# 5l1v3r1/PBS

Measured on AMD Instinct MI355X. Metric: co-run slowdown (%) vs solo + aggregate throughput, 4-tenant mix at 1/2/4/8 GPU, higher is better.
Workload: dtype bf16

## Files before the change

csrc/hip/tenant_kernels.hip:

```cpp
#include "common.hpp"

namespace gpbs_hip {


__device__ __forceinline__ int grab_unit_x(WorkQueue* q, const PartTable* table, u32 mode, u32 me, u32 xcc,
                                           int* s_slot, u32 total) {
  if (threadIdx.x == 0) {
    int u = -1;
    hold_wait(table, mode);
    const u32 per = (total + kXcds - 1) / kXcds;
    for (u32 spins = 0;; ++spins) {
      if (owns(table, mode, me, xcc)) {
        for (u32 k = 0; k < (u32)kXcds; ++k) {
          const u32 r = (xcc + k) & (kXcds - 1);
          const u32 lo = r * per, hi = min(lo + per, total);
          if (lo >= hi) continue;
          if (__hip_atomic_load(&q->xnext[r], __ATOMIC_RELAXED, __HIP_MEMORY_SCOPE_AGENT) >= hi - lo) continue;
          const u32 t = atomicAdd(&q->xnext[r], 1u);
          if (t < hi - lo) {
            u = (int)(lo + t);
            atomicAdd(&q->next, 1u);
            break;
          }
        }
        break;
      }
      if ((mode & 3) != GATE_PARK || spins >= kParkSpins ||
          __hip_atomic_load(&q->next, __ATOMIC_RELAXED, __HIP_MEMORY_SCOPE_AGENT) >= total) {
        atomicAdd(&q->stopped, 1u);
        break;
      }
#pragma unroll
      for (int k = 0; k < 6; ++k) __builtin_amdgcn_s_sleep(127);
    }
    *s_slot = u;
  }
  __syncthreads();
  int u = *s_slot;
  __syncthreads();
  return u;
}


__device__ __forceinline__ u16 f2bf(float x) { return __builtin_bit_cast(u16, (__bf16)x); }
__device__ __forceinline__ float bf2f(u16 x) { return __uint_as_float(((u32)x) << 16); }

constexpr int GBM = 128, GBN = 128, GBK = 64, GNT = 256;
constexpr int kGemmLds = 2 * 2 * GBM * GBK * 2;

typedef __attribute__((address_space(3))) char lds_t;

__device__ __forceinline__ void glds16(const void* g, lds_t* l) {
  __builtin_amdgcn_global_load_lds(g, (__attribute__((address_space(3))) void*)l, 16, 0, 0);
}

__global__ __launch_bounds__(GNT, 2) void k_gemm_bf16_tn(const u16* __restrict__ A, const u16* __restrict__ Bt,
                                                         u16* __restrict__ C, int M, int N, int K, WorkQueue* q,
                                                         const PartTable* table, u32 mode, u32 me, u64* cnt,
                                                         u32 inst_per_tile, u32 refs_per_tile, u32 miss_per_tile,
                                                         u32* status) {
  __shared__ __attribute__((aligned(16))) char smem[kGemmLds + 16];
  lds_t* lds = (lds_t*)smem;
  int* s_slot = (int*)(smem + kGemmLds);
  const u32 xcc = xcc_id();
  u64 t_last = __builtin_amdgcn_s_memtime();
  const int tid = threadIdx.x, lane = tid & 63, wid = tid >> 6;
  const int wr = wid >> 1, wc = wid & 1;
  const int tiles_m = M / GBM, tiles_n = N / GBN, ntiles = tiles_m * tiles_n;
  const int nk = K / GBK;
  constexpr int GROUP_M = 8;

  int srow[4], scol[4];
#pragma unroll
  for (int j = 0; j < 4; ++j) {
    const int c = wid * 4 + j;
    srow[j] = 8 * c + (lane >> 3);
    scol[j] = (((lane & 7) ^ (srow[j] & 7)) * 8);
  }

  for (;;) {
    const int t = grab_unit(q, table, mode, me, xcc, s_slot, (u32)ntiles);
    if (t < 0) break;
    const int in_group = GROUP_M * tiles_n;
    const int g = t / in_group;
    const int first_m = g * GROUP_M;
    const int gsz = min(tiles_m - first_m, GROUP_M);
    const int tm = first_m + (t % in_group) % gsz;
    const int tn = (t % in_group) / gsz;
    const u16* Ab = A + (size_t)tm * GBM * K;
    const u16* Bb = Bt + (size_t)tn * GBN * K;

    f32x4 acc[4][4];
#pragma unroll
    for (int i = 0; i < 4; ++i)
#pragma unroll
      for (int j = 0; j < 4; ++j) acc[i][j] = f32x4{0.f, 0.f, 0.f, 0.f};

    auto stage = [&](int buf, int kt) {
      lds_t* la = lds + buf * (2 * GBM * GBK * 2);
      lds_t* lb = la + GBM * GBK * 2;
#pragma unroll
      for (int j = 0; j < 4; ++j) {
        const int c = wid * 4 + j;
        glds16(Ab + (size_t)srow[j] * K + kt * GBK + scol[j], la + c * 1024);
        glds16(Bb + (size_t)srow[j] * K + kt * GBK + scol[j], lb + c * 1024);
      }
    };

    stage(0, 0);
    asm volatile("s_waitcnt vmcnt(0)" ::: "memory");
    __syncthreads();
    int cur = 0;
    for (int kt = 0; kt < nk; ++kt) {
      if (kt + 1 < nk) stage(cur ^ 1, kt + 1);
      const lds_t* la = lds + cur * (2 * GBM * GBK * 2);
      const lds_t* lb = la + GBM * GBK * 2;
#pragma unroll
      for (int s = 0; s < 2; ++s) {
        bf16x8 a[4], b[4];
        const int chunk = s * 4 + (lane >> 4);
#pragma unroll
        for (int i = 0; i < 4; ++i) {
          const int ra = wr * 64 + i * 16 + (lane & 15);
          a[i] = *(const __attribute__((address_space(3))) bf16x8*)(la + ra * 128 + ((chunk ^ (ra & 7)) << 4));
          const int rb = wc * 64 + i * 16 + (lane & 15);
          b[i] = *(const __attribute__((address_space(3))) bf16x8*)(lb + rb * 128 + ((chunk ^ (rb & 7)) << 4));
        }
#pragma unroll
        for (int i = 0; i < 4; ++i)
#pragma unroll
          for (int j = 0; j < 4; ++j) acc[i][j] = __builtin_amdgcn_mfma_f32_16x16x32_bf16(a[i], b[j], acc[i][j], 0, 0, 0);
      }
      asm volatile("s_waitcnt vmcnt(0)" ::: "memory");
      __syncthreads();
      cur ^= 1;
    }
#pragma unroll
    for (int i = 0; i < 4; ++i)
#pragma unroll
      for (int j = 0; j < 4; ++j) {
        const int m = tm * GBM + wr * 64 + i * 16 + (lane >> 4) * 4;
        const int n = tn * GBN + wc * 64 + j * 16 + (lane & 15);
#pragma unroll
        for (int r = 0; r < 4; ++r) C[(size_t)(m + r) * N + n] = f2bf(acc[i][j][r]);
      }
    count_unit(cnt, me, xcc, inst_per_tile, &t_last, refs_per_tile, miss_per_tile, q);
  }
  finish(q, status, (u32)ntiles);
}

constexpr int G2_BM = 256, G2_BK = 64, G2_NT = 512;
constexpr u32 kGemmXRange = 1u << 16;
constexpr u32 kGemmBlock2D = 1u << 17;
constexpr u32 kGemmStatic = 1u << 18;
constexpr int kGemmOptsLive = 1 | 8 | 1 << 23;
constexpr int kGemmOptsShipped = 256 | 8192 | 65536 | 131072;
static int g_gemm_opts = 8;
constexpr int kG2Half = 128 * 128;
constexpr int kG2Buf = 4 * kG2Half;
constexpr int kG2Lds = 2 * kG2Buf;

__device__ __forceinline__ int g2_swz(int r) { return (r >> 1) & 7; }

__global__ __launch_bounds__(G2_NT, 1) void k_gemm256_bf16_tn(const u16* __restrict__ A, const u16* __restrict__ Bt,
                                                             u16* __restrict__ C, int M, int N, int K, WorkQueue* q,
                                                             const PartTable* table, u32 mode, u32 me, u64* cnt,
                                                             u32 inst_per_tile, u32 refs_per_tile, u32 miss_per_tile,
                                                             u32* status) {
  __shared__ __attribute__((aligned(16))) char smem[kG2Lds + 16];
  lds_t* lds = (lds_t*)smem;
  int* s_slot = (int*)(smem + kG2Lds);
  const u32 xcc = xcc_id();
  u64 t_last = __builtin_amdgcn_s_memtime();
  const int tid = threadIdx.x, lane = tid & 63, wid = tid >> 6;
  const int wu = __builtin_amdgcn_readfirstlane(wid);
  const int wr = wu >> 2, wc = wu & 3;
  const int tiles_m = M / G2_BM, tiles_n = N / G2_BM, ntiles = tiles_m * tiles_n;
  const int nt = K / G2_BK;
  int soff[2];
#pragma unroll
  for (int j = 0; j < 2; ++j) {
    const int row = 8 * (2 * wid + j) + (lane >> 3);
    soff[j] = row * K + (((lane & 7) ^ g2_swz(row)) * 8);
  }
  int soffa[4];
#pragma unroll
  for (int j = 0; j < 4; ++j) {
    const int row = 8 * (4 * (wid & 3) + j) + (lane >> 3);
    soffa[j] = row * K + (((lane & 7) ^ g2_swz(row)) * 8);
  }
  const int l16 = lane & 15, lq = lane >> 4;
  const int bh = wc >> 1, bc = (wc & 1) * 64;
  int units_seen = 0;

  for (;;) {
    const int tile = (mode & kGemmStatic) ? (units_seen ? -1 : (int)blockIdx.x)
                     : (mode & kGemmXRange) ? grab_unit_x(q, table, mode, me, xcc, s_slot, (u32)ntiles)
                                            : grab_unit(q, table, mode, me, xcc, s_slot, (u32)ntiles);
    if (tile < 0) break;
    int tm = tile / tiles_n, tn = tile % tiles_n;
    if ((mode & kGemmBlock2D) && (tiles_m & 3) == 0 && (tiles_n & 1) == 0 && ntiles % kXcds == 0) {
      const int per = ntiles / kXcds;
      const int bm = tiles_m / 4, bn = tiles_n / 2;
      const int g = (mode & kGemmXRange) ? tile / per : tile % kXcds;
      const int jj = (mode & kGemmXRange) ? tile % per : tile / kXcds;
      tm = (g >> 1) * bm + jj / bn;
      tn = (g & 1) * bn + jj % bn;
    }
    const u16* Ab = A + (size_t)tm * G2_BM * K;
    const u16* Bb = Bt + (size_t)tn * G2_BM * K;
    auto stage = [&](int kind, int h, int t) {
      const u16* src = (kind ? Bb : Ab) + (size_t)h * 128 * K + t * G2_BK;
      lds_t* dst = lds + (t & 1) * kG2Buf + (kind * 2 + h) * kG2Half + wid * 2048;
      glds16(src + soff[0], dst);
      glds16(src + soff[1], dst + 1024);
    };
    auto stage_own_a = [&](int t) {
      const u16* src = Ab + (size_t)wr * 128 * K + t * G2_BK;
      lds_t* dst = lds + (t & 1) * kG2Buf + wr * kG2Half + (wid & 3) * 4096;
#pragma unroll
      for (int j = 0; j < 4; ++j) glds16(src + soffa[j], dst + j * 1024);
    };
    auto frag = [&](int b, int kind, int h, int r0, int s) -> bf16x8 {
      const int r = r0 + l16;
      const lds_t* p = lds + b * kG2Buf + (kind * 2 + h) * kG2Half + r * 128 + (((4 * s + lq) ^ g2_swz(r)) << 4);
      return *(const __attribute__((address_space(3))) bf16x8*)p;
    };
    f32x4 acc[8][4];
#pragma unroll
    for (int i = 0; i < 8; ++i)
#pragma unroll
      for (int j = 0; j < 4; ++j) acc[i][j] = f32x4{0.f, 0.f, 0.f, 0.f};
    stage(1, 0, 0); stage(1, 1, 0); stage(0, 0, 0); stage(0, 1, 0);
    asm volatile("s_waitcnt vmcnt(0)" ::: "memory");
    __builtin_amdgcn_s_barrier();
    if (wr == 1) __builtin_amdgcn_s_barrier();
    bf16x8 a[4][2], b[4][2];
    for (int t = 0; t < nt; ++t) {
      const int buf = t & 1;
      const bool more = t + 1 < nt;
#pragma unroll
      for (int j = 0; j < 4; ++j)
#pragma unroll
        for (int s2 = 0; s2 < 2; ++s2) b[j][s2] = frag(buf, 1, bh, bc + j * 16, s2);
      __builtin_amdgcn_sched_barrier(0);
#pragma unroll
      for (int i = 0; i < 4; ++i)
#pragma unroll
        for (int s2 = 0; s2 < 2; ++s2) a[i][s2] = frag(buf, 0, wr, i * 16, s2);
      if (more) {
        stage(1, 0, t + 1); stage(1, 1, t + 1);
      } else {
        asm volatile("s_waitcnt vmcnt(0)" ::: "memory");
      }
      __builtin_amdgcn_s_barrier();
      asm volatile("s_waitcnt lgkmcnt(0)" ::: "memory");
      __builtin_amdgcn_s_setprio(1);
#pragma unroll
      for (int s2 = 0; s2 < 2; ++s2)
#pragma unroll
        for (int i = 0; i < 4; ++i)
#pragma unroll
          for (int j = 0; j < 4; ++j)
            acc[i][j] = __builtin_amdgcn_mfma_f32_16x16x32_bf16(b[j][s2], a[i][s2], acc[i][j], 0, 0, 0);
      __builtin_amdgcn_s_setprio(0);
      __builtin_amdgcn_s_barrier();
#pragma unroll
      for (int i = 0; i < 4; ++i)
#pragma unroll
        for (int s2 = 0; s2 < 2; ++s2) a[i][s2] = frag(buf, 0, wr, 64 + i * 16, s2);
      if (more) {
        stage_own_a(t + 1);
        asm volatile("s_waitcnt vmcnt(4)" ::: "memory");
      }
      __builtin_amdgcn_s_barrier();
      asm volatile("s_waitcnt lgkmcnt(0)" ::: "memory");
      __builtin_amdgcn_s_setprio(1);
#pragma unroll
      for (int s2 = 0; s2 < 2; ++s2)
#pragma unroll
        for (int i = 0; i < 4; ++i)
#pragma unroll
          for (int j = 0; j < 4; ++j)
            acc[4 + i][j] = __builtin_amdgcn_mfma_f32_16x16x32_bf16(b[j][s2], a[i][s2], acc[4 + i][j], 0, 0, 0);
      __builtin_amdgcn_s_setprio(0);
      asm volatile("s_waitcnt vmcnt(0)" ::: "memory");
      __builtin_amdgcn_s_barrier();
    }
    if (wr == 0) __builtin_amdgcn_s_barrier();
#pragma unroll
    for (int i = 0; i < 8; ++i)
#pragma unroll
      for (int j = 0; j < 4; ++j) {
        const int m = wr * 128 + i * 16 + l16;
        const int c8 = wc * 16 + j * 4 + lq;
        const u32 lo = (u32)f2bf(acc[i][j][0]) | ((u32)f2bf(acc[i][j][1]) << 16);
        const u32 hi = (u32)f2bf(acc[i][j][2]) | ((u32)f2bf(acc[i][j][3]) << 16);
        *(__attribute__((address_space(3))) u32x2*)(lds + m * 512 + ((c8 ^ (m & 15)) << 3)) = u32x2{lo, hi};
      }
    __syncthreads();
#pragma unroll
    for (int p = 0; p < 16; ++p) {
      const int row = p * 16 + (tid >> 5), c16 = tid & 31;
      u32x4 v = *(const __attribute__((address_space(3))) u32x4*)(lds + row * 512 + (((2 * c16) ^ (row & 14)) << 3));
      if (row & 1) v = u32x4{v.z, v.w, v.x, v.y};
      u32x4* dst = (u32x4*)(C + (size_t)(tm * G2_BM + row) * N + tn * G2_BM + c16 * 8);
      __builtin_nontemporal_store(v, dst);
    }
    __syncthreads();
    ++units_seen;
    if (!(mode & kGemmStatic)) count_unit(cnt, me, xcc, inst_per_tile, &t_last, refs_per_tile, miss_per_tile, q);
  }
  if (!(mode & kGemmStatic)) finish(q, status, (u32)ntiles);
}

constexpr int SNT = 256, SUNROLL = 16, RUNROLL = 6;

template <int U, bool NTS>
__global__ __launch_bounds__(SNT) void k_stream_copy(const f32x4* __restrict__ src, f32x4* __restrict__ dst,
                                                    u64 n4, u32 chunk4, WorkQueue* q, const PartTable* table, u32 mode,
                                                    u32 me, u64* cnt, u32* status) {
  __shared__ int s_slot[4];
  const u32 xcc = xcc_id();
  u64 t_last = __builtin_amdgcn_s_memtime();
  const u32 nchunks = (u32)((n4 + chunk4 - 1) / chunk4);
  const u64 lines = (u64)chunk4 * 16 / 128;
  const u64 inst = (u64)chunk4 * 2 / 64 + 8;
  for (;;) {
    const int c = grab_unit(q, table, mode, me, xcc, s_slot, nchunks);
    if (c < 0) break;
    const u64 base = (u64)c * chunk4;
    const u64 end = min(base + chunk4, n4);
    for (u64 i = base + threadIdx.x; i < end; i += (u64)SNT * U) {
      f32x4 v[U];
#pragma unroll
      for (int k = 0; k < U; ++k) {
        const u64 idx = i + (u64)k * SNT;
        if (idx < end) v[k] = __builtin_nontemporal_load(src + idx);
      }
#pragma unroll
      for (int k = 0; k < U; ++k) {
        const u64 idx = i + (u64)k * SNT;
        if (idx < end) {
          if constexpr (NTS)
            __builtin_nontemporal_store(v[k], dst + idx);
          else
            dst[idx] = v[k];
        }
      }
    }
    count_unit(cnt, me, xcc, inst, &t_last, 2 * lines, 2 * lines, q);
  }
  finish(q, status, nchunks);
}

template <int NT, int U, bool NTL, bool NTS>
__global__ __launch_bounds__(NT) void k_reduce_bf16(const u32x4* __restrict__ a, const u32x4* __restrict__ b,
                                                    u32x4* __restrict__ out, u64 n8, u32 chunk8, WorkQueue* q,
                                                    const PartTable* table, u32 mode, u32 me, u64* cnt,
                                                    u32* status) {
  __shared__ int s_slot[4];
  const u32 xcc = xcc_id();
  u64 t_last = __builtin_amdgcn_s_memtime();
  const u32 nchunks = (u32)((n8 + chunk8 - 1) / chunk8);
  const u64 lines = (u64)chunk8 * 16 / 128;
  const u64 inst = (u64)chunk8 * 3 / 64 + (u64)chunk8 * 16 / 64;
  for (;;) {
    const int c = grab_unit(q, table, mode, me, xcc, s_slot, nchunks);
    if (c < 0) break;
    const u64 base = (u64)c * chunk8, end = min(base + chunk8, n8);
    for (u64 i = base + threadIdx.x; i < end; i += (u64)NT * U) {
      u32x4 x[U], y[U];
#pragma unroll
      for (int k = 0; k < U; ++k) {
        const u64 idx = i + (u64)k * NT;
        if (idx < end) {
          if constexpr (NTL) {
            x[k] = __builtin_nontemporal_load(a + idx);
            y[k] = __builtin_nontemporal_load(b + idx);
          } else {
            x[k] = a[idx];
            y[k] = b[idx];
          }
        }
      }
#pragma unroll
      for (int k = 0; k < U; ++k) {
        const u64 idx = i + (u64)k * NT;
        if (idx >= end) continue;
        const u32* px = (const u32*)&x[k];
        const u32* py = (const u32*)&y[k];
        u32x4 r;
        u32* pr = (u32*)&r;
#pragma unroll
        for (int w = 0; w < 4; ++w) {
          const float lo = bf2f((u16)(px[w] & 0xffff)) + bf2f((u16)(py[w] & 0xffff));
          const float hi = bf2f((u16)(px[w] >> 16)) + bf2f((u16)(py[w] >> 16));
          pr[w] = (u32)f2bf(lo) | ((u32)f2bf(hi) << 16);
        }
        if constexpr (NTS)
          __builtin_nontemporal_store(r, out + idx);
        else
          out[idx] = r;
      }
    }
    count_unit(cnt, me, xcc, inst, &t_last, 3 * lines, 3 * lines, q);
  }
  finish(q, status, nchunks);
}

constexpr int GV_U = 2;

__device__ __forceinline__ float dot8(const u32x4 w, const u32x4 v) {
  float s = 0.f;
#pragma unroll
  for (int e = 0; e < 4; ++e) {
    s += __uint_as_float(w[e] << 16) * __uint_as_float(v[e] << 16);
    s += __uint_as_float(w[e] & 0xffff0000u) * __uint_as_float(v[e] & 0xffff0000u);
  }
  return s;
}

__global__ __launch_bounds__(256) __attribute__((amdgpu_waves_per_eu(5, 8))) void k_gemv_bf16(const u16* __restrict__ W, const u16* __restrict__ x,
                                                  float* __restrict__ y, int R, int K, WorkQueue* q,
                                                  const PartTable* table, u32 mode, u32 me, u64* cnt,
                                                  u32* status) {
  __shared__ int s_slot[4];
  if (mode & GATE_WAVEPRIO) __builtin_amdgcn_s_setprio(3);
  const u32 xcc = xcc_id();
  u64 t_last = __builtin_amdgcn_s_memtime();
  const int lane = threadIdx.x & 63, wid = threadIdx.x >> 6;
  const u32 nchunks = (u32)((R + 15) / 16);
  const u64 lines = (u64)16 * K * 2 / 128;
  const int nk = K / 512;
  const u32x4* xv = (const u32x4*)x;
  for (;;) {
    const int c = grab_unit(q, table, mode, me, xcc, s_slot, nchunks);
    if (c < 0) break;
    const int row0 = c * 16 + wid * 4;
    const u32x4* wr[4];
#pragma unroll
    for (int r = 0; r < 4; ++r) wr[r] = (const u32x4*)(W + (size_t)min(row0 + r, R - 1) * K);
    float acc[4] = {0.f, 0.f, 0.f, 0.f};
    int kc = 0;
    for (; kc + GV_U <= nk; kc += GV_U) {
      u32x4 xr[GV_U], wv[GV_U][4];
#pragma unroll
      for (int u = 0; u < GV_U; ++u) {
        const int k = (kc + u) * 64 + lane;
        xr[u] = xv[k];
#pragma unroll
        for (int r = 0; r < 4; ++r) wv[u][r] = __builtin_nontemporal_load(wr[r] + k);
      }
#pragma unroll
      for (int u = 0; u < GV_U; ++u)
#pragma unroll
        for (int r = 0; r < 4; ++r) acc[r] += dot8(wv[u][r], xr[u]);
    }
    for (; kc < nk; ++kc) {
      const int k = kc * 64 + lane;
      const u32x4 xr = xv[k];
#pragma unroll
      for (int r = 0; r < 4; ++r) acc[r] += dot8(__builtin_nontemporal_load(wr[r] + k), xr);
    }
#pragma unroll
    for (int r = 0; r < 4; ++r) {
      float s = acc[r];
#pragma unroll
      for (int off = 32; off > 0; off >>= 1) s += __shfl_xor(s, off, 64);
      if (lane == 0 && row0 + r < R) y[row0 + r] = s;
    }
    count_unit(cnt, me, xcc, (u64)16 * (K / 512 + 8), &t_last, lines, lines, q);
  }
  finish(q, status, nchunks);
}

__global__ void k_census(u32* out, const PartTable* table, u32 mode, u32 me) {
  const u32 xcc = xcc_id();
  const bool ok = owns(table, mode, me, xcc);
  if (threadIdx.x == 0) {
    out[blockIdx.x * 4 + 0] = xcc;
    out[blockIdx.x * 4 + 1] = hw_id();
    out[blockIdx.x * 4 + 2] = ok ? 1u : 0u;
    out[blockIdx.x * 4 + 3] = 0xC0FFEEu;
  }
  if (ok) {
    u64 t = __builtin_amdgcn_s_memtime();
    while (__builtin_amdgcn_s_memtime() - t < 2000) __builtin_amdgcn_s_sleep(1);
  }
}

}

using namespace gpbs_hip;

extern "C" {

int gpbs_hip_set_gemm_opts(int opts) {
  const int old = g_gemm_opts;
  if (opts < 0) return old;
  const int gone = opts & ~(kGemmOptsLive | kGemmOptsShipped);
  static bool warned = false;
  if (gone && !warned) {
    warned = true;
    fprintf(stderr,
            "gpbs_hip_set_gemm_opts: bits 0x%x select GEMM variants that were removed (docs/gemm_lab.md); "
            "the shipped schedule runs\n",
            gone);
  }
  g_gemm_opts = opts & kGemmOptsLive;
  return old;
}

int gpbs_hip_gemm_units(int M, int N) {
  if (M % G2_BM == 0 && N % G2_BM == 0) return (M / G2_BM) * (N / G2_BM);
  return (M / GBM) * (N / GBN);
}

int gpbs_hip_gemm_bf16(const void* A, const void* Bt, void* C, int M, int N, int K, void* q, const void* table,
                       unsigned mode, unsigned me, void* cnt, void* status, int grid, hipStream_t s) {
  if (M % GBM || N % GBN || K % GBK || M <= 0 || N <= 0 || K <= 0) return -22;
  if (M % G2_BM == 0 && N % G2_BM == 0) {
    const int ntiles = (M / G2_BM) * (N / G2_BM);
    if (grid <= 0) grid = 256;
    if (grid > ntiles) grid = ntiles;
    const u32 inst = (u32)((G2_BM / 16) * (G2_BM / 16) * (K / 32) + (K / G2_BK) * 64 + 128);
    const u32 refs = (u32)(((u64)2 * G2_BM * K * 2) / 128);
    const u32 miss = (u32)((((u64)M + N) * K * 2 / 128) / ntiles + (u64)G2_BM * G2_BM * 2 / 128);
    const u32 m2 = mode | ((g_gemm_opts & 1) ? kGemmXRange : 0u) |
                   ((g_gemm_opts & 8) && ntiles % kXcds == 0 ? kGemmBlock2D : 0u) |
                   ((g_gemm_opts & (1 << 23)) && (mode & 3) == GATE_NONE && grid == ntiles ? kGemmStatic : 0u);
    hipLaunchKernelGGL(k_gemm256_bf16_tn, dim3(grid), dim3(G2_NT), 0, s, (const u16*)A, (const u16*)Bt, (u16*)C, M, N,
                       K, (WorkQueue*)q, (const PartTable*)table, m2, me, (u64*)cnt, inst, refs, miss, (u32*)status);
    return hipGetLastError() == hipSuccess ? 0 : -5;
  }
  const int ntiles = (M / GBM) * (N / GBN);
  if (grid <= 0) grid = 256 * 2;
  if (grid > ntiles) grid = ntiles;
  const u32 inst = (u32)((GBM / 16) * (GBN / 16) * (K / 32) * 2 + (K / GBK) * 32 + 64);
  const u32 refs = (u32)(((u64)(GBM + GBN) * K * 2) / 128);
  const u32 miss = (u32)((((u64)M + N) * K * 2 / 128) / ntiles + (u64)GBM * GBN * 2 / 128);
  hipLaunchKernelGGL(k_gemm_bf16_tn, dim3(grid), dim3(GNT), 0, s, (const u16*)A, (const u16*)Bt, (u16*)C, M, N, K,
                     (WorkQueue*)q, (const PartTable*)table, mode, me, (u64*)cnt, inst, refs, miss, (u32*)status);
  return hipGetLastError() == hipSuccess ? 0 : -5;
}

static int g_stream_opts = 0;

int gpbs_hip_set_stream_opts(int opts) {
  const int old = g_stream_opts;
  if (opts >= 0) g_stream_opts = opts;
  return old;
}

int gpbs_hip_stream_copy(const void* src, void* dst, unsigned long long bytes, unsigned chunk_bytes, void* q,
                         const void* table, unsigned mode, unsigned me, void* cnt, void* status, int grid, hipStream_t s) {
  if (bytes % 16 || chunk_bytes % 16 || chunk_bytes == 0) return -22;
  if (grid <= 0) grid = 256;
  using K = void (*)(const f32x4*, f32x4*, u64, u32, WorkQueue*, const PartTable*, u32, u32, u64*, u32*);
  static const K tab[4] = {k_stream_copy<SUNROLL, true>, k_stream_copy<SUNROLL, false>, k_stream_copy<8, true>,
                           k_stream_copy<8, false>};
  hipLaunchKernelGGL(tab[g_stream_opts & 3], dim3(grid), dim3(SNT), 0, s, (const f32x4*)src, (f32x4*)dst, bytes / 16,
                     chunk_bytes / 16, (WorkQueue*)q, (const PartTable*)table, mode, me, (u64*)cnt, (u32*)status);
  return hipGetLastError() == hipSuccess ? 0 : -5;
}

static int g_reduce_opts = 8;

int gpbs_hip_set_reduce_opts(int opts) {
  const int old = g_reduce_opts;
  if (opts >= 0) g_reduce_opts = opts;
  return old;
}

int gpbs_hip_reduce_bf16(const void* a, const void* b, void* out, unsigned long long bytes, unsigned chunk_bytes,
                         void* q, const void* table, unsigned mode, unsigned me, void* cnt, void* status, int grid, hipStream_t s) {
  if (bytes % 16 || chunk_bytes % 16 || chunk_bytes == 0) return -22;
  if (grid <= 0) grid = 256;
  using K = void (*)(const u32x4*, const u32x4*, u32x4*, u64, u32, WorkQueue*, const PartTable*, u32, u32, u64*, u32*);
#define RV(NT, U) {k_reduce_bf16<NT, U, true, true>, k_reduce_bf16<NT, U, false, true>, \
                   k_reduce_bf16<NT, U, true, false>, k_reduce_bf16<NT, U, false, false>}
  static const K table256[4][4] = {RV(256, 6), RV(256, 8), RV(256, 4), RV(256, 12)};
  static const K table512[4][4] = {RV(512, 6), RV(512, 8), RV(512, 4), RV(512, 12)};
#undef RV
  const int o = g_reduce_opts;
  const int nt = (o & 16) ? 512 : 256;
  const K kern = ((o & 16) ? table512 : table256)[o & 3][((o >> 2) & 1) | (((o >> 3) & 1) << 1)];
  hipLaunchKernelGGL(kern, dim3(grid), dim3(nt), 0, s, (const u32x4*)a, (const u32x4*)b, (u32x4*)out,
                     bytes / 16, chunk_bytes / 16, (WorkQueue*)q, (const PartTable*)table, mode, me, (u64*)cnt, (u32*)status);
  return hipGetLastError() == hipSuccess ? 0 : -5;
}

int gpbs_hip_gemv_bf16(const void* W, const void* x, void* y, int R, int K, void* q, const void* table, unsigned mode,
                       unsigned me, void* cnt, void* status, int grid, hipStream_t s) {
  if (K % 512 || R <= 0) return -22;
  if (grid <= 0) grid = (R + 15) / 16;
  if (grid > 256) grid = 256;
  hipLaunchKernelGGL(k_gemv_bf16, dim3(grid), dim3(256), 0, s, (const u16*)W, (const u16*)x, (float*)y, R, K,
                     (WorkQueue*)q, (const PartTable*)table, mode, me, (u64*)cnt, (u32*)status);
  return hipGetLastError() == hipSuccess ? 0 : -5;
}

int gpbs_hip_census(void* out, int blocks, const void* table, unsigned mode, unsigned me, hipStream_t s) {
  hipLaunchKernelGGL(k_census, dim3(blocks), dim3(64), 0, s, (u32*)out, (const PartTable*)table, mode, me);
  return hipGetLastError() == hipSuccess ? 0 : -5;
}

}
```

pbs_amd/ops/hipabi.py:

```python
from __future__ import annotations

import ctypes as C

from .. import _native as N

u32, i32, u64, i64 = C.c_uint32, C.c_int32, C.c_uint64, C.c_int64
vp = C.c_void_p


class RunnerCfg(C.Structure):
    _fields_ = [(n, C.c_int) for n in ("kind", "tenant", "gate", "priority", "depth", "grid", "M", "N", "K",
                                       "chunk_bytes", "engine_wake", "reserved")] + \
               [("bytes", C.c_ulonglong), ("a", vp), ("b", vp), ("c", vp)] + \
               [(n, C.c_int) for n in ("alt_kind", "alt_M", "alt_N", "alt_K", "alt_chunk_bytes", "alt_reserved")] + \
               [("alt_bytes", C.c_ulonglong), ("alt_a", vp), ("alt_b", vp), ("alt_c", vp)]


class RunnerStats(C.Structure):
    _fields_ = [(n, u64) for n in ("units_done", "launches", "relaunches", "waits_owner", "submitted")] + \
               [(n, i64) for n in ("busy_ns", "wait_owner_ns", "first_start_ns", "last_done_ns", "lat_sum_ns",
                                   "lat_max_ns")] + [("lat_count", u64), ("units_alt", u64)] + \
               [("drain_sum_ns", i64), ("drain_max_ns", i64), ("drain_count", u64)]


KIND = {"gemm": 1, "stream": 2, "reduce": 3, "gemv": 4, "allreduce": 5, "gemm_fp8": 6}


def _p(lib, name, res, *args):
    f = getattr(lib, name)
    f.restype = res
    f.argtypes = list(args)


def bind(lib):
    _p(lib, "gpbs_roctx_push", C.c_int, C.c_char_p)
    _p(lib, "gpbs_roctx_pop", C.c_int)
    _p(lib, "gpbs_roctx_mark", None, C.c_char_p)
    _p(lib, "gpbs_gpu_switch_latency", C.c_int, vp, C.c_int, C.c_int, vp)
    _p(lib, "gpbs_hip_gemm_bf16", C.c_int, vp, vp, vp, C.c_int, C.c_int, C.c_int, vp, vp, C.c_uint, C.c_uint, vp, vp,
       C.c_int, vp)
    _p(lib, "gpbs_hip_gemm_fp8", C.c_int, vp, vp, vp, vp, vp, C.c_int, C.c_int, C.c_int, C.c_int, vp, vp, C.c_uint,
       C.c_uint, vp, vp, C.c_int, vp)
    _p(lib, "gpbs_hip_gemm_fp8_units", C.c_int, C.c_int, C.c_int)
    _p(lib, "gpbs_hip_stream_copy", C.c_int, vp, vp, C.c_ulonglong, C.c_uint, vp, vp, C.c_uint, C.c_uint, vp, vp,
       C.c_int, vp)
    _p(lib, "gpbs_hip_reduce_bf16", C.c_int, vp, vp, vp, C.c_ulonglong, C.c_uint, vp, vp, C.c_uint, C.c_uint, vp, vp,
       C.c_int, vp)
    _p(lib, "gpbs_hip_gemv_bf16", C.c_int, vp, vp, vp, C.c_int, C.c_int, vp, vp, C.c_uint, C.c_uint, vp, vp, C.c_int,
       vp)
    _p(lib, "gpbs_hip_set_gemm_opts", C.c_int, C.c_int)
    _p(lib, "gpbs_hip_set_reduce_opts", C.c_int, C.c_int)
    _p(lib, "gpbs_hip_set_stream_opts", C.c_int, C.c_int)
    _p(lib, "gpbs_hwc_init", C.c_int, C.c_char_p)
    _p(lib, "gpbs_hwc_init_gpu", C.c_int, C.c_char_p, C.c_int)
    _p(lib, "gpbs_hwc_start", C.c_int)
    _p(lib, "gpbs_hwc_active", C.c_int)
    _p(lib, "gpbs_hwc_trace_enable", C.c_int, C.c_int)
    _p(lib, "gpbs_hwc_trace_stats", C.c_int, C.c_char_p, C.c_int, C.c_int)
    _p(lib, "gpbs_hwc_sample", C.c_int, C.POINTER(C.c_uint64), C.c_int)
    _p(lib, "gpbs_hwc_stop", C.c_int)
    _p(lib, "gpbs_gpu_set_hwc", C.c_int, vp, C.c_int)
    _p(lib, "gpbs_gpu_hwc_stats", C.c_int, vp, C.POINTER(C.c_uint64), C.POINTER(C.c_uint64), C.POINTER(C.c_double))
    _p(lib, "gpbs_hwc_sample_se", C.c_int, C.POINTER(C.c_uint64), C.POINTER(C.c_uint64))
    _p(lib, "gpbs_hwc_slot_per_se", C.c_int, C.c_int)
    _p(lib, "gpbs_hwc_agent", C.c_int, C.c_char_p, C.c_int, C.POINTER(C.c_int))
    _p(lib, "gpbs_gpu_hwc_period", C.c_int, vp, C.c_int, C.c_int, C.POINTER(C.c_uint64))
    _p(lib, "gpbs_gpu_hwc_quality", C.c_int, vp, C.POINTER(C.c_uint64), C.POINTER(C.c_double), C.POINTER(C.c_int))
    _p(lib, "gpbs_gpu_hwc_tenant", C.c_int, vp, C.c_int, C.POINTER(C.c_double), C.POINTER(C.c_double))
    _p(lib, "gpbs_gpu_hwc_reset", C.c_int, vp)
    _p(lib, "gpbs_gpu_hwc_clean", C.c_int, vp, C.c_int, C.POINTER(C.c_double))
    _p(lib, "gpbs_gpu_hwc_tenant_metric", C.c_int, vp, C.c_int, C.POINTER(C.c_double))
    _p(lib, "gpbs_gpu_set_share", C.c_int, vp, C.c_int, C.POINTER(C.c_int64))
    _p(lib, "gpbs_gpu_hwc_poll", C.c_int, vp)
    _p(lib, "gpbs_gpu_set_se_mode", C.c_int, vp, C.c_int)
    _p(lib, "gpbs_hip_rmsnorm_bf16", C.c_int, vp, vp, vp, C.c_int, C.c_int, C.c_float, vp)
    _p(lib, "gpbs_hip_swiglu_bf16", C.c_int, vp, vp, vp, C.c_ulonglong, vp)
    _p(lib, "gpbs_hip_quant_rows_fp8", C.c_int, vp, vp, vp, C.c_int, C.c_int, vp)
    _p(lib, "gpbs_hip_rmsnorm_quant_fp8", C.c_int, vp, vp, vp, vp, C.c_int, C.c_int, C.c_float, vp)
    _p(lib, "gpbs_hip_swiglu_quant_fp8", C.c_int, vp, vp, vp, C.c_int, C.c_int, vp)
    _p(lib, "gpbs_hip_fp8_set_opts", C.c_int, C.c_int)
    _p(lib, "gpbs_hip_fp8_linear_res", C.c_int, vp, vp, vp, vp, vp, vp, C.c_int, C.c_int, C.c_int, vp)
    _p(lib, "gpbs_hip_fp8_linear", C.c_int, vp, vp, vp, vp, vp, C.c_int, C.c_int, C.c_int, vp)
    _p(lib, "gpbs_hip_rope_bf16_dpos", C.c_int, vp, vp, vp, vp, C.c_int, C.c_int, C.c_int, C.c_int, vp, vp)
    _p(lib, "gpbs_hip_qkv_rope_cache", C.c_int, vp, vp, vp, vp, vp, vp, vp, C.c_int, C.c_int, C.c_int, C.c_int,
       C.c_int, vp)
    _p(lib, "gpbs_hip_decode_attn", C.c_int, vp, vp, vp, vp, vp, vp, C.c_int, C.c_int, C.c_int, C.c_int, C.c_int,
       C.c_int, C.c_float, vp)
    _p(lib, "gpbs_hip_qkv_rope_cache_prefill", C.c_int, vp, vp, vp, vp, vp, vp, C.c_int, C.c_int, C.c_int, C.c_int,
       C.c_int, C.c_int, C.c_int, vp)
    _p(lib, "gpbs_hip_prefill_attn", C.c_int, vp, vp, vp, vp, C.c_int, C.c_int, C.c_int, C.c_int, C.c_int, C.c_int,
       C.c_int, C.c_float, vp)
    _p(lib, "gpbs_hip_qkv_rope_cache_seq", C.c_int, vp, vp, vp, vp, vp, vp, vp, C.c_int, C.c_int, C.c_int, C.c_int,
       C.c_int, vp)
    _p(lib, "gpbs_hip_decode_attn_seq", C.c_int, vp, vp, vp, vp, vp, vp, C.c_int, C.c_int, C.c_int, C.c_int, C.c_int,
       C.c_int, C.c_float, vp)
    _p(lib, "gpbs_hip_qkv_rope_cache_prefill_seq", C.c_int, vp, vp, vp, vp, vp, vp, vp, vp, C.c_int, C.c_int, C.c_int,
       C.c_int, C.c_int, C.c_int, vp)
    _p(lib, "gpbs_hip_prefill_attn_seq", C.c_int, vp, vp, vp, vp, vp, vp, C.c_int, C.c_int, C.c_int, C.c_int, C.c_int,
       C.c_int, C.c_float, vp)
    _p(lib, "gpbs_hip_qkv_rope_cache_paged", C.c_int, vp, vp, vp, vp, vp, vp, vp, vp, C.c_int, C.c_int, C.c_int,
       C.c_int, C.c_int, C.c_int, C.c_int, vp)
    _p(lib, "gpbs_hip_decode_attn_paged", C.c_int, vp, vp, vp, vp, vp, vp, vp, C.c_int, C.c_int, C.c_int, C.c_int,
       C.c_int, C.c_int, C.c_int, C.c_int, C.c_float, vp)
    _p(lib, "gpbs_hip_qkv_rope_cache_prefill_paged", C.c_int, vp, vp, vp, vp, vp, vp, vp, vp, vp, C.c_int, C.c_int,
       C.c_int, C.c_int, C.c_int, C.c_int, C.c_int, C.c_int, vp)
    _p(lib, "gpbs_hip_prefill_attn_paged", C.c_int, vp, vp, vp, vp, vp, vp, vp, C.c_int, C.c_int, C.c_int, C.c_int,
       C.c_int, C.c_int, C.c_int, C.c_int, C.c_float, vp)
    _p(lib, "gpbs_hip_qkv_rope_cache_paged_kv8", C.c_int, vp, vp, vp, vp, vp, vp, vp, vp, vp, vp, C.c_int, C.c_int,
       C.c_int, C.c_int, C.c_int, C.c_int, C.c_int, vp)
    _p(lib, "gpbs_hip_decode_attn_paged_kv8", C.c_int, vp, vp, vp, vp, vp, vp, vp, vp, vp, C.c_int, C.c_int, C.c_int,
       C.c_int, C.c_int, C.c_int, C.c_int, C.c_int, C.c_float, vp)
    _p(lib, "gpbs_hip_qkv_rope_cache_prefill_paged_kv8", C.c_int, vp, vp, vp, vp, vp, vp, vp, vp, vp, vp, vp, C.c_int,
       C.c_int, C.c_int, C.c_int, C.c_int, C.c_int, C.c_int, C.c_int, vp)
    _p(lib, "gpbs_hip_prefill_attn_paged_kv8", C.c_int, vp, vp, vp, vp, vp, vp, vp, vp, vp, C.c_int, C.c_int, C.c_int,
       C.c_int, C.c_int, C.c_int, C.c_int, C.c_int, C.c_float, vp)
    _p(lib, "gpbs_hip_rope_bf16", C.c_int, vp, vp, vp, vp, C.c_int, C.c_int, C.c_int, C.c_int, C.c_int, vp)
    _p(lib, "gpbs_hip_census", C.c_int, vp, C.c_int, vp, C.c_uint, C.c_uint, vp)
    _p(lib, "gpbs_hip_partition_switch", C.c_int, vp, C.c_uint, C.POINTER(C.c_uint), vp)
    _p(lib, "gpbs_hip_counter_reduce", C.c_int, vp, vp, vp, C.c_int, vp, vp)
    _p(lib, "gpbs_hip_adapt", C.c_int, vp, vp, vp, vp, C.c_int, vp, vp, vp)
    _p(lib, "gpbs_gpu_ctx_create", vp, C.c_int, C.c_int, C.c_int, C.c_int)
    _p(lib, "gpbs_gpu_set_nctx", C.c_int, vp, C.c_int)
    _p(lib, "gpbs_gpu_set_table_mode", C.c_int, vp, C.c_int)
    _p(lib, "gpbs_gpu_table_mode", C.c_int, vp)
    _p(lib, "gpbs_gpu_set_hold", C.c_int, vp, C.c_int, C.POINTER(C.c_uint64))
    _p(lib, "gpbs_gpu_force_hold", C.c_int, vp, C.c_int)
    _p(lib, "gpbs_gpu_set_spatial", C.c_int, vp, C.c_int)
    _p(lib, "gpbs_gpu_set_waveprio", C.c_int, vp, C.c_int)
    _p(lib, "gpbs_gpu_set_lat_half", C.c_int, vp, C.c_int)
    _p(lib, "gpbs_gpu_hwc_attr_stats", C.c_int, vp, C.POINTER(u64), C.POINTER(u64), C.POINTER(u64))
    _p(lib, "gpbs_gpu_set_hwc_device", C.c_int, vp, C.c_int)
    _p(lib, "gpbs_gpu_hwc_duty", C.c_int, vp, C.c_int, C.POINTER(u64))
    _p(lib, "gpbs_gpu_hwc_bursts", C.c_int, vp, C.POINTER(u64), C.POINTER(u64))
    _p(lib, "gpbs_gpu_hwc_budget_stats", C.c_int, vp, C.POINTER(u64))
    _p(lib, "gpbs_gpu_hwc_sampler", C.c_int, vp, C.c_int, C.c_int, C.c_int)
    _p(lib, "gpbs_gpu_param", C.c_int, vp, C.c_char_p, C.c_int)
    _p(lib, "gpbs_gpu_hwc_attr_timing", C.c_int, vp, C.POINTER(u64))
    _p(lib, "gpbs_gpu_hwc_measure_reqs", C.c_uint64, vp)
    _p(lib, "gpbs_gpu_hwc_align", C.c_int, vp, C.c_int, C.c_int, C.c_int, C.POINTER(u64))
    _p(lib, "gpbs_gpu_hwc_tenant_periods", C.c_int, vp, C.c_int, C.POINTER(u64), C.POINTER(C.c_double))
    _p(lib, "gpbs_gpu_switch_cost", C.c_int, vp, C.c_int, C.POINTER(i64))
    _p(lib, "gpbs_gpu_hwc_tenant_cadence", C.c_int, vp, C.c_int, C.POINTER(i64))
    _p(lib, "gpbs_gpu_cadence_ring", C.c_int, vp, C.POINTER(i64), C.c_int)
    _p(lib, "gpbs_gpu_block_probe", C.c_int, vp, C.c_int, C.c_int, C.c_int, C.c_int, C.POINTER(i64))
    _p(lib, "gpbs_runner_queue", C.c_int, vp)
    _p(lib, "gpbs_gpu_masked_pool", C.c_int, C.POINTER(C.c_uint64), C.c_int)
    _p(lib, "gpbs_hip_masked_pool_selftest", C.c_int)
    _p(lib, "gpbs_hip_hwc_fold_selftest", C.c_int)
    _p(lib, "gpbs_hip_hwc_drained_selftest", C.c_int, C.c_int, C.c_int)
    _p(lib, "gpbs_hip_hwc_cadence_selftest", C.c_int)
    _p(lib, "gpbs_hip_masked_pool_prealloc", C.c_int, C.c_int, C.POINTER(C.c_int), C.c_int)
    _p(lib, "gpbs_gpu_adapt_stats", C.c_int, vp, C.POINTER(u64), C.POINTER(u64), C.POINTER(u64))
    _p(lib, "gpbs_hip_hwc_attr_selftest", C.c_int, C.c_int, C.c_int, C.POINTER(C.c_double))
    _p(lib, "gpbs_hip_hwc_attr_host_check", C.c_int, C.c_int, C.c_int, C.POINTER(C.c_double))
    _p(lib, "gpbs_hip_hwc_attr_bench", C.c_int, C.c_int, C.POINTER(C.c_double))
    _p(lib, "gpbs_hip_adapt_pools_selftest", C.c_int, C.c_int)
    _p(lib, "gpbs_gpu_ctx_destroy", None, vp)
    _p(lib, "gpbs_gpu_attach", C.c_int, vp, vp, C.c_int, C.c_int)
    _p(lib, "gpbs_gpu_backend_ops", C.c_int, vp, vp, C.POINTER(N.ActuatorOps), C.POINTER(N.CounterOps), C.c_int)
    _p(lib, "gpbs_gpu_table", vp, vp)
    _p(lib, "gpbs_gpu_counters", vp, vp)
    _p(lib, "gpbs_gpu_set_owners", C.c_int, vp, C.POINTER(C.c_int))
    _p(lib, "gpbs_gpu_get_owners", C.c_int, vp, C.POINTER(C.c_int))
    _p(lib, "gpbs_gpu_read_counters", C.c_int, vp, C.c_int, C.POINTER(u64), C.POINTER(u64))
    _p(lib, "gpbs_gpu_stats", C.c_int, vp, C.POINTER(u64))
    _p(lib, "gpbs_gpu_ownership", C.c_int, vp, C.c_int, C.POINTER(i64), C.c_int)
    _p(lib, "gpbs_gpu_cumask_stream", vp, C.c_int, C.POINTER(C.c_uint32), C.c_int, C.c_int)
    _p(lib, "gpbs_gpu_stream_destroy", C.c_int, vp)
    _p(lib, "gpbs_runner_create", vp, vp, C.POINTER(RunnerCfg))
    _p(lib, "gpbs_runner_submit", C.c_int, vp, C.c_int)
    _p(lib, "gpbs_runner_wait", C.c_int, vp, i64)
    _p(lib, "gpbs_runner_stats", C.c_int, vp, C.POINTER(RunnerStats))
    _p(lib, "gpbs_runner_latencies", C.c_int, vp, C.POINTER(i64), C.c_int, C.c_int)
    _p(lib, "gpbs_runner_reset_stats", C.c_int, vp)
    _p(lib, "gpbs_runner_set_gate", C.c_int, vp, C.c_int)
    _p(lib, "gpbs_runner_cancel", i64, vp)
    _p(lib, "gpbs_runner_set_engine_wake", C.c_int, vp, C.c_int)
    _p(lib, "gpbs_runner_stream", vp, vp)
    _p(lib, "gpbs_runner_set_phase", C.c_int, vp, C.c_int)
    _p(lib, "gpbs_coll_create", vp, C.c_int, C.c_int, C.c_int, C.c_ulonglong)
    _p(lib, "gpbs_coll_export", C.c_int, vp, vp)
    _p(lib, "gpbs_coll_handle_bytes", C.c_int)
    _p(lib, "gpbs_coll_open", C.c_int, vp, C.c_int, vp)
    _p(lib, "gpbs_coll_finalize", C.c_int, vp)
    _p(lib, "gpbs_coll_buffer", vp, vp, C.c_int)
    _p(lib, "gpbs_coll_destroy", None, vp)
    _p(lib, "gpbs_gangx_create", vp, C.c_int, C.c_int, C.c_int, C.c_int)
    _p(lib, "gpbs_gangx_handle_bytes", C.c_int)
    _p(lib, "gpbs_gangx_export", C.c_int, vp, vp)
    _p(lib, "gpbs_gangx_open", C.c_int, vp, C.c_int, vp)
    _p(lib, "gpbs_gangx_finalize", C.c_int, vp)
    _p(lib, "gpbs_gangx_exchange", C.c_int, vp, C.c_uint, C.POINTER(C.c_longlong), C.c_int,
       C.POINTER(C.c_longlong), C.c_longlong)
    _p(lib, "gpbs_gangx_stats", C.c_int, vp, C.POINTER(u64))
    _p(lib, "gpbs_gangx_destroy", None, vp)
    _p(lib, "gpbs_coll_copy", C.c_int, vp, C.c_int, vp, C.c_ulonglong, C.c_int)
    _p(lib, "gpbs_runner_destroy", None, vp)
```

Measured before the change: 1.256.

## Swizzle GEMM tiles within XCD blocks and make XRange stealing sticky

Moves the per-XCD block tile mapping into a shared header. Inside each XCD block it walks tiles in 2x2/4x4 supertiles instead of row-major order, aiming for better L2 reuse of A and B panels. The XRange grabber now remembers the last range it stole from, so it does not rescan its home range every time. It also stops early once the global count is exhausted, and disables the static path when a status buffer is passed. A host helper exports the tile map for inspection. The cost is extra index arithmetic per tile and some change to atomic contention patterns.

```diff
diff --git a/csrc/hip/gemm_tile_map.hpp b/csrc/hip/gemm_tile_map.hpp
--- /dev/null
+++ b/csrc/hip/gemm_tile_map.hpp
@@ -0,0 +1,44 @@
+#pragma once
+#include <hip/hip_runtime.h>
+
+namespace gpbs_hip {
+
+constexpr int kTileMapXcds = 8;
+
+__host__ __device__ inline bool gemm_blocks_apply(int tiles_m, int tiles_n) {
+  return (tiles_m & 3) == 0 && (tiles_n & 1) == 0 && (tiles_m * tiles_n) % kTileMapXcds == 0;
+}
+
+__host__ __device__ inline void gemm_block_walk(int jj, int bm, int bn, int& r, int& c) {
+  if (((bm | bn) & 3) == 0) {
+    const int sb = jj >> 4, k = jj & 15, sbn = bn >> 2;
+    r = (sb / sbn) * 4 + ((k >> 3) & 1) * 2 + ((k >> 1) & 1);
+    c = (sb % sbn) * 4 + ((k >> 2) & 1) * 2 + (k & 1);
+  } else if (((bm | bn) & 1) == 0) {
+    const int qd = jj >> 2, qn = bn >> 1;
+    r = (qd / qn) * 2 + ((jj >> 1) & 1);
+    c = (qd % qn) * 2 + (jj & 1);
+  } else {
+    r = jj / bn;
+    c = jj % bn;
+  }
+}
+
+__host__ __device__ inline void gemm_tile_map(int tile, int tiles_m, int tiles_n, bool block2d, bool xrange, int& tm,
+                                              int& tn) {
+  if (!block2d) {
+    tm = tile / tiles_n;
+    tn = tile % tiles_n;
+    return;
+  }
+  const int per = tiles_m * tiles_n / kTileMapXcds;
+  const int bm = tiles_m / 4, bn = tiles_n / 2;
+  const int g = xrange ? tile / per : tile % kTileMapXcds;
+  const int jj = xrange ? tile % per : tile / kTileMapXcds;
+  int r, c;
+  gemm_block_walk(jj, bm, bn, r, c);
+  tm = (g >> 1) * bm + r;
+  tn = (g & 1) * bn + c;
+}
+
+}
diff --git a/csrc/hip/tenant_kernels.hip b/csrc/hip/tenant_kernels.hip
--- a/csrc/hip/tenant_kernels.hip
+++ b/csrc/hip/tenant_kernels.hip
@@ -1,4 +1,5 @@
 #include "common.hpp"
+#include "gemm_tile_map.hpp"
 
 namespace gpbs_hip {
 
@@ -11,17 +12,21 @@
     const u32 per = (total + kXcds - 1) / kXcds;
     for (u32 spins = 0;; ++spins) {
       if (owns(table, mode, me, xcc)) {
+        const u32 cur = (u32)s_slot[1] & (kXcds - 1);
         for (u32 k = 0; k < (u32)kXcds; ++k) {
-          const u32 r = (xcc + k) & (kXcds - 1);
+          const u32 r = (cur + k) & (kXcds - 1);
           const u32 lo = r * per, hi = min(lo + per, total);
-          if (lo >= hi) continue;
-          if (__hip_atomic_load(&q->xnext[r], __ATOMIC_RELAXED, __HIP_MEMORY_SCOPE_AGENT) >= hi - lo) continue;
-          const u32 t = atomicAdd(&q->xnext[r], 1u);
-          if (t < hi - lo) {
-            u = (int)(lo + t);
-            atomicAdd(&q->next, 1u);
-            break;
+          const u32 claimed = k ? 0u : __hip_atomic_load(&q->next, __ATOMIC_RELAXED, __HIP_MEMORY_SCOPE_AGENT);
+          if (lo < hi) {
+            const u32 t = atomicAdd(&q->xnext[r], 1u);
+            if (t < hi - lo) {
+              u = (int)(lo + t);
+              atomicAdd(&q->next, 1u);
+              if (k) s_slot[1] = (int)r;
+              break;
+            }
           }
+          if (k == 0 && claimed >= total) break;
         }
         break;
       }
@@ -192,21 +197,16 @@
   const int l16 = lane & 15, lq = lane >> 4;
   const int bh = wc >> 1, bc = (wc & 1) * 64;
   int units_seen = 0;
+  if (tid == 0) s_slot[1] = (int)xcc;
+  const bool block2d = (mode & kGemmBlock2D) && gemm_blocks_apply(tiles_m, tiles_n);
 
   for (;;) {
     const int tile = (mode & kGemmStatic) ? (units_seen ? -1 : (int)blockIdx.x)
                      : (mode & kGemmXRange) ? grab_unit_x(q, table, mode, me, xcc, s_slot, (u32)ntiles)
                                             : grab_unit(q, table, mode, me, xcc, s_slot, (u32)ntiles);
     if (tile < 0) break;
-    int tm = tile / tiles_n, tn = tile % tiles_n;
-    if ((mode & kGemmBlock2D) && (tiles_m & 3) == 0 && (tiles_n & 1) == 0 && ntiles % kXcds == 0) {
-      const int per = ntiles / kXcds;
-      const int bm = tiles_m / 4, bn = tiles_n / 2;
-      const int g = (mode & kGemmXRange) ? tile / per : tile % kXcds;
-      const int jj = (mode & kGemmXRange) ? tile % per : tile / kXcds;
-      tm = (g >> 1) * bm + jj / bn;
-      tn = (g & 1) * bn + jj % bn;
-    }
+    int tm, tn;
+    gemm_tile_map(tile, tiles_m, tiles_n, block2d, (mode & kGemmXRange) != 0, tm, tn);
     const u16* Ab = A + (size_t)tm * G2_BM * K;
     const u16* Bb = Bt + (size_t)tn * G2_BM * K;
     auto stage = [&](int kind, int h, int t) {
@@ -517,6 +517,15 @@
   return (M / GBM) * (N / GBN);
 }
 
+int gpbs_hip_gemm_tile_map(int M, int N, int opts, int* tm_tn) {
+  if (M <= 0 || N <= 0 || M % G2_BM || N % G2_BM || !tm_tn) return -22;
+  const int tiles_m = M / G2_BM, tiles_n = N / G2_BM, ntiles = tiles_m * tiles_n;
+  const bool block2d = (opts & 8) && ntiles % kXcds == 0 && gemm_blocks_apply(tiles_m, tiles_n);
+  for (int t = 0; t < ntiles; ++t)
+    gemm_tile_map(t, tiles_m, tiles_n, block2d, (opts & 1) != 0, tm_tn[2 * t], tm_tn[2 * t + 1]);
+  return ntiles;
+}
+
 int gpbs_hip_gemm_bf16(const void* A, const void* Bt, void* C, int M, int N, int K, void* q, const void* table,
                        unsigned mode, unsigned me, void* cnt, void* status, int grid, hipStream_t s) {
   if (M % GBM || N % GBN || K % GBK || M <= 0 || N <= 0 || K <= 0) return -22;
@@ -529,7 +538,8 @@
     const u32 miss = (u32)((((u64)M + N) * K * 2 / 128) / ntiles + (u64)G2_BM * G2_BM * 2 / 128);
     const u32 m2 = mode | ((g_gemm_opts & 1) ? kGemmXRange : 0u) |
                    ((g_gemm_opts & 8) && ntiles % kXcds == 0 ? kGemmBlock2D : 0u) |
-                   ((g_gemm_opts & (1 << 23)) && (mode & 3) == GATE_NONE && grid == ntiles ? kGemmStatic : 0u);
+                   ((g_gemm_opts & (1 << 23)) && (mode & 3) == GATE_NONE && grid == ntiles && !status ? kGemmStatic
+                                                                                                       : 0u);
     hipLaunchKernelGGL(k_gemm256_bf16_tn, dim3(grid), dim3(G2_NT), 0, s, (const u16*)A, (const u16*)Bt, (u16*)C, M, N,
                        K, (WorkQueue*)q, (const PartTable*)table, m2, me, (u64*)cnt, inst, refs, miss, (u32*)status);
     return hipGetLastError() == hipSuccess ? 0 : -5;
diff --git a/pbs_amd/ops/hipabi.py b/pbs_amd/ops/hipabi.py
--- a/pbs_amd/ops/hipabi.py
+++ b/pbs_amd/ops/hipabi.py
@@ -49,6 +49,7 @@
     _p(lib, "gpbs_hip_gemv_bf16", C.c_int, vp, vp, vp, C.c_int, C.c_int, vp, vp, C.c_uint, C.c_uint, vp, vp, C.c_int,
        vp)
     _p(lib, "gpbs_hip_set_gemm_opts", C.c_int, C.c_int)
+    _p(lib, "gpbs_hip_gemm_tile_map", C.c_int, C.c_int, C.c_int, C.c_int, vp)
     _p(lib, "gpbs_hip_set_reduce_opts", C.c_int, C.c_int)
     _p(lib, "gpbs_hip_set_stream_opts", C.c_int, C.c_int)
     _p(lib, "gpbs_hwc_init", C.c_int, C.c_char_p)
```

New measurement: 1.244. 1.0% lower.
